# archi-physics/archi

Hardware: AMD Instinct MI355X
Metric: kNN queries/sec @ top-10, 10M x 768 bf16 corpus (higher is better)
Workload: dtype bf16

## Files before the change

### archi_amd/_lib.py

```python
from __future__ import annotations

import ctypes
import os
import threading

_HERE = os.path.dirname(os.path.abspath(__file__))
LIB_PATH = os.path.join(_HERE, "lib", "libarchi_hip.so")

DTYPES = {"f32": 0, "bf16": 1, "f16": 2}
METRICS = {"cosine": 0, "l2": 1, "inner_product": 2}
SEARCH_MODES = {"auto": 0, "exact": 1, "fast_only": 2}
POOLING = {"mean": 0, "cls": 1, "last": 2}


class HipBackendError(RuntimeError):
    """Raised when the HIP backend is unavailable or a call fails."""


class StaleFilterError(HipBackendError):
    """A search was handed a row_filter built for another layout of the index (AK_ERR_STALE_FILTER): a writer added rows
    or reclaimed tombstones between the mask's construction and the search. Rebuild the mask and retry."""


ERR_STALE_FILTER = -11
# ... 164 lines not shown
    ("ak_index_generate", _I, [_P, _U64, _U32, _U64, _I64, _I, _I64]),
    ("ak_index_remove", _I, [_P, _P, _I64, ctypes.POINTER(_I64)]),
    ("ak_index_count", _I, [_P, ctypes.POINTER(_I64)]),
    ("ak_index_fetch", _I, [_P, _P, _I64, _P]),
    ("ak_index_lookup", _I, [_P, _P, _I64, _P]),
    ("ak_index_distances", _I, [_P, _P, _P, _I64, _P, _P]),
    ("ak_index_search", _I, [_P, _P, _I, _I, _I, _P, _I64, _U64, _P, _P, _P, _P]),
    ("ak_index_lex_attach", _I, [_P, _P, _I64, _P, _P, _P, _P, _U64]),
    ("ak_index_lex_clear", _I, [_P, _U64]),
    ("ak_index_lex_info", _I, [_P, ctypes.POINTER(_U64), ctypes.POINTER(_I64), ctypes.POINTER(_I64), ctypes.POINTER(_I64)]),
    ("ak_index_lex_scores", _I, [_P, _P, _I, _D, _D, _D, _P, _P, _P]),
    ("ak_index_hybrid_search", _I, [_P, _P, _P, _I, _D, _D, _D, _D, _D, _P, _I64, _P, _I64, _U64, _I, _P, _P, ctypes.POINTER(_I),
                                    _P, _P, ctypes.POINTER(_I), _P]),
    ("ak_index_search_dev", _I, [_P, _P, _I, _I, _I, _P, _I64, _U64, _P, _P, _P, _P]),
    ("ak_index_slots", _I, [_P, ctypes.POINTER(_I64), ctypes.POINTER(_I64), ctypes.POINTER(_U64)]),
    ("ak_index_compact", _I, [_P, ctypes.POINTER(_I64)]),
    ("ak_index_scan_plan", _I, [_P, _I, _I, _P]),
    ("ak_index_i8_info", _I, [_P, _P]),
    ("ak_index_debug_read", _I, [_P, _P, _I]),
    ("ak_index_profile", _I, [_P, _I]),
    ("ak_index_profile_read", _I, [_P, _P, _I, ctypes.POINTER(_I)]),
    ("ak_merge_topk_dev", _I, [_I, _I, _I, _P, _P, _P, _P, _P]),
    ("ak_merge_shards_dev", _I, [_I, _I, _I, _P, _I64, _P, _P, _P, _P]),
    ("ak_comm_unique_id", _I, [_P]),
    ("ak_comm_create", _I, [_P, _I, _I, ctypes.POINTER(_P)]),
    ("ak_comm_destroy", _I, [_P]),
    ("ak_index_search_sharded_dev", _I, [_P, _P, _P, _I, _I, _P, _I64, _U64, _P, _P, ctypes.POINTER(_I64), _P]),
    ("ak_shard_payload_begin_dev", _I, [_P, _I, _I, _P]),
    ("ak_shard_fail_payload_dev", _I, [_P, _I, _I, _I, _P]),
    ("ak_shard_status_dev", _I, [_I, _P, _I64, _P, _P]),
    ("ak_shard_gather_rows_dev", _I, [_P, _P, _I, _I, _P, _P]),
    ("ak_shard_scatter_topk_dev", _I, [_P, _I, _I, _P, _P, _P, _P, _P]),
    ("ak_l2_normalize_dev", _I, [_P, _I64, _I, _P]),
    ("ak_encoder_create", _I, [ctypes.POINTER(AkBertConfig), _P, _I, ctypes.POINTER(_P)]),
    ("ak_encoder_destroy", _I, [_P]),
    ("ak_encoder_forward", _I, [_P, _P, _P, _I, _I, _I, _I, _P, _P]),
    ("ak_encoder_forward_lens", _I, [_P, _P, _I, _P, _I, _I, _I, _I, _I, _P, _P]),
    ("ak_encoder_gelu_table", _I, [_P]),
    ("ak_encoder_set_rel_bias", _I, [_P, _P, _I, _I]),
    ("ak_encoder_set_positions_from_ids", _I, [_P, _I, _I]),
    ("ak_decoder_create", _I, [ctypes.POINTER(AkDecoderConfig), _P, _I, ctypes.POINTER(_P)]),
    ("ak_decoder_destroy", _I, [_P]),
    ("ak_decoder_forward_lens", _I, [_P, _P, _I, _P, _I, _I, _I, _I, _P, _P]),
    ("ak_decoder_rope_table", _I, [ctypes.c_float, _I, _I, _P, _P]),
    ("ak_decoder_rope_table_inv", _I, [_P, _I, _I, _P, _P]),
    ("ak_mbert_create", _I, [ctypes.POINTER(AkModernBertConfig), _P, _I, ctypes.POINTER(_P)]),
    ("ak_mbert_destroy", _I, [_P]),
    ("ak_mbert_forward_lens", _I, [_P, _P, _I, _P, _I, _I, _I, _I, _I, _P, _P]),
    ("ak_gemma_create", _I, [ctypes.POINTER(AkGemmaConfig), _P, _I, ctypes.POINTER(_P)]),
    ("ak_gemma_destroy", _I, [_P]),
    ("ak_gemma_set_rope_inv_freq", _I, [_P, _P, _P]),
    ("ak_gemma_forward_lens", _I, [_P, _P, _I, _P, _I, _I, _I, _I, _I, _P, _P]),
    ("ak_nomic_create", _I, [ctypes.POINTER(AkNomicBertConfig), _P, _I, ctypes.POINTER(_P)]),
    ("ak_nomic_destroy", _I, [_P]),
    ("ak_nomic_forward_lens", _I, [_P, _P, _I, _P, _I, _I, _I, _I, _I, _P, _P]),
    ("ak_t5_create", _I, [ctypes.POINTER(AkT5Config), _P, _I, ctypes.POINTER(_P)]),
    ("ak_t5_destroy", _I, [_P]),
    ("ak_t5_forward_lens", _I, [_P, _P, _I, _P, _I, _I, _I, _I, _I, _P, _P]),
    ("ak_llama_create", _I, [ctypes.POINTER(AkLlamaConfig), _P, _I, ctypes.POINTER(_P)]),
    ("ak_llama_destroy", _I, [_P]),
    ("ak_llama_set_rope_inv_freq", _I, [_P, _P]),
    ("ak_llama_forward_lens", _I, [_P, _P, _I, _P, _I, _I, _I, _I, _I, _P, _P]),
    ("ak_qwen2_create", _I, [ctypes.POINTER(AkQwen2Config), _P, _I, ctypes.POINTER(_P)]),
    ("ak_qwen2_destroy", _I, [_P]),
    ("ak_qwen2_set_rope_inv_freq", _I, [_P, _P]),
    ("ak_qwen2_forward_lens", _I, [_P, _P, _I, _P, _I, _I, _I, _I, _I, _P, _P]),
    ("ak_wordpiece_create", _I, [ctypes.c_char_p, _I, ctypes.POINTER(_P)]),
    ("ak_wordpiece_create_ex", _I, [ctypes.c_char_p, _I, ctypes.c_char_p, ctypes.c_char_p, ctypes.c_char_p,
                                    ctypes.POINTER(ctypes.c_char_p), _I, ctypes.POINTER(_P)]),
    ("ak_wordpiece_destroy", _I, [_P]),
    ("ak_wordpiece_encode", _I, [_P, _P, _P, _I64, _I, _I, _P, _P]),
]


class AkKtGemm(ctypes.Structure):
    _fields_ = [
        ("X", _P), ("W", _P), ("bias", _P),
        ("T", _I), ("N", _I), ("K", _I),
        ("out_bf16", _P), ("ldo", _I),
        ("out_f32", _P),
        ("res16", _P),
        ("q", _P), ("k", _P), ("vt", _P), ("H", _I), ("S", _I), ("qscale", ctypes.c_float),
    ]


class AkKtGemmLazy(ctypes.Structure):
    _fields_ = [
        ("X", _P), ("W", _P), ("bias", _P),
        ("T", _I), ("N", _I), ("K", _I),
        ("out_bf16", _P), ("ldo", _I),
        ("res16", _P),
        ("q", _P), ("k", _P), ("vt", _P), ("H", _I), ("S", _I), ("qscale", ctypes.c_float),
        ("fold_c", _P), ("a_stats", _P), ("res_stats", _P), ("res_g", _P), ("res_b", _P), ("out_g", _P),
        ("out_stats", _P),
        ("nslot", _I), ("inv_h", ctypes.c_float), ("eps", ctypes.c_float),
    ]


KT_SYMBOLS = [
    ("ak_kt_attn", _I, [_P, _P, _P, _P, _P, _I, _I, _I, _I, _I, _I, _P, _P, _P, _I, _P]),
    ("ak_kt_attn_long", _I, [_P, _P, _P, _P, _P, _P, _I, _I, _I, _I, _I, _I, _P]),
    ("ak_kt_attn_window", _I, [_P, _P, _P, _P, _P, _P, _I, _I, _I, _I, _I, _I, _I, _P]),
    ("ak_kt_attn_causal", _I, [_P, _P, _P, _P, _P, _I, _I, _I, _I, _P]),
    ("ak_kt_gemm", _I, [_I, ctypes.POINTER(AkKtGemm), _P]),
    ("ak_kt_gemm_skinny", _I, [_P, _P, _P, _I, _I, _I, _P, _P, _I, _P]),
    ("ak_kt_gemm_skinny_qkv", _I, [_P, _P, _P, _I, _I, _I, _P, _P, _P, _I, _I, ctypes.c_float, _P]),
    ("ak_kt_vt_pos", _I, [_I]),
    ("ak_kt_gemm_ln", _I, [_P, _P, _P, _P, _P, _P, _P, _I, _I, ctypes.c_float, _P]),
    ("ak_kt_ffn384_weight_bytes", _I64, [_I]),
    ("ak_kt_ffn384", _I, [_P] * 13 + [_I, _I, ctypes.c_float, _P]),
    ("ak_kt_qkv384_weight_bytes", _I64, []),
    ("ak_kt_qkv384", _I, [_P] * 7 + [_I, _I, _I, ctypes.c_float, _I, _P]),
    ("ak_kt_gemm_lazy", _I, [_I, ctypes.POINTER(AkKtGemmLazy), _P]),
    ("ak_kt_ln_finalize", _I, [_P, _I, _I64, ctypes.c_float, ctypes.c_float, _P, _P]),
    ("ak_kt_fold_ln", _I, [_P, _P, _P, _P, _I, _I, _P, _P, _P]),
    ("ak_kt_layernorm", _I, [_P, _P, _P, _P, _P, _I, _I, ctypes.c_float, _P, _P, _P, _P]),
    ("ak_kt_layernorm16", _I, [_P, _P, _P, _I, _I, ctypes.c_float, _P, _P]),
    ("ak_kt_ln_apply16", _I, [_P, _P, _P, _P, _I64, _I, _P, _P]),
]

KTG_SYMBOLS = [
    ("ak_ktg_attn_gqa", _I, [_P, _P, _P, _P, _P, _I, _I, _I, _I, _I, _P]),
    ("ak_ktg_qk_norm_rope", _I, [_P, _I, _I, _I, _I, _P, _P, ctypes.c_float, _P, _P, ctypes.c_float, _P, _P, _P, _P]),
    ("ak_ktg_gemm_geglu_tanh", _I, [_P, _P, _P, _I, _I, _I, _P, _P]),
]

_F = ctypes.c_float
_EMBED = [_P, _I, _P, _I, _I, _I, _I, _I, _P, _P, _F, _P, _P]
KTS_SYMBOLS = [
    ("ak_kts_dec_embed", _I, _EMBED + [_P, _P]),
    ("ak_kts_dec_add_rmsnorm", _I, [_P, _P, _I64, _I, _P, _F, _P, _P]),
    ("ak_kts_dec_qk_rope", _I, [_P, _I, _I, _I, _I, _P, _P, _F, _P, _P, _F, _P, _P, _P, _P]),
    ("ak_kts_dec_pool", _I, [_P, _P, _I, _I, _I, _P, _F, _I, _P, _P]),
    ("ak_kts_mb_embed", _I, _EMBED + [_P, _P, _P]),
    ("ak_kts_mb_add_ln", _I, [_P, _P, _I64, _I, _P, _F, _P, _P]),
    ("ak_kts_mb_rope", _I, [_P, _P, _I64, _I, _I, _P, _P, _P]),
    ("ak_kts_mb_pool", _I, [_P, _P, _I, _I, _I, _F, _P, _I, _I, _P, _P, _P]),
    ("ak_kts_nb_embed", _I, [_P, _I, _P, _I, _I, _I, _I, _I, _P, _P, _P, _P, _F, _P, _P, _P, _P, _P]),
    ("ak_kts_nb_add_ln", _I, [_P, _P, _I64, _I, _P, _P, _F, _P, _P]),
    ("ak_kts_nb_pool", _I, [_P, _P, _I, _I, _I, _I, _I, _P, _P, _P]),
    ("ak_kts_gm_fold1p", _I, [_P, _I, _P, _P]),
    ("ak_kts_gm_embed", _I, _EMBED + [_P, _P]),
    ("ak_kts_gm_norm_add_norm", _I, [_P, _P, _I64, _I, _P, _P, _F, _P, _P, _P]),
    ("ak_kts_gm_pool", _I, [_P, _P, _I, _I, _I, _P, _P, _P]),
    ("ak_kts_gm_dense", _I, [_P, _P, _I, _I, _I, _P, _P]),
    ("ak_kts_gm_l2", _I, [_P, _I, _I, _I, _P, _P]),
    ("ak_kts_gemm_bf16", _I, [_P, _P, _P, _I, _I, _I, _P, _P]),
    ("ak_kts_ll_attn", _I, [_P, _P, _P, _P, _P, _I, _I, _I, _I, _I, _I, _P]),
    ("ak_kts_ll_pool", _I, [_P, _P, _I, _I, _I, _P, _F, _I, _P, _P, _P]),
    ("ak_kts_ll_rope", _I, [_P, _I, _I, _I, _I, _P, _P, _F, _P, _P, _P, _P]),
    ("ak_kts_q2_attn", _I, [_P, _P, _P, _P, _P, _I, _I, _I, _I, _I, _P]),
    ("ak_kts_t5_attn", _I, [_P, _P, _P, _P, _P, _P, _I, _I, _I, _I, _I, _I, _P, _I, _P]),
    ("ak_kts_t5_gemm_relu", _I, [_P, _P, _P, _I, _I, _I, _P, _P]),
]


def load() -> ctypes.CDLL:
    global _lib
    with _lock:
        if _lib is None:
            import torch
            path = LIB_PATH
            if os.environ.get("ARCHI_HIP_DBG") or any(os.environ.get(v) for v in DBG_SWITCHES) or \
                    os.environ.get("AK_SCAN_CFG", "")[:1] in ("X", "O") or os.environ.get("AK_ATTN_STREAM", "") in ("3", "4"):
                dbg = os.path.join(_HERE, "lib", "libarchi_hip_dbg.so")
                if not os.path.exists(dbg):
                    raise HipBackendError(f"{dbg} not found: the instrumented kernels are built by `make -C archi_amd/csrc dbg`")
                path = dbg
            if not os.path.exists(LIB_PATH):
                raise HipBackendError(
                    f"{LIB_PATH} not found: build it with `make -C archi_amd/csrc` "
                    "(or __graft_entry__.build()); archi_amd has no CPU fallback")
            lib = ctypes.CDLL(path)
            for name, res, args in SYMBOLS:
                fn = getattr(lib, name)
                fn.restype = res
                fn.argtypes = args
            if path != LIB_PATH:
                for name, res, args in KT_SYMBOLS + KTG_SYMBOLS + KTS_SYMBOLS:
                    fn = getattr(lib, name)
                    fn.restype = res
                    fn.argtypes = args
            got = lib.ak_abi_version()
            if got != ABI_VERSION:
                raise HipBackendError(f"{path}: ABI version {got}, this binding expects {ABI_VERSION} "
                                      "(rebuild with `make -C archi_amd/csrc`; signatures moved between the two)")
            _lib = lib
    return _lib


def is_dbg_library() -> bool:
    lib = load()
    return bool(getattr(lib, "_name", "").endswith("libarchi_hip_dbg.so"))


def debug_set(name: str, value: str | None) -> None:
    check(load().ak_debug_set(name.encode(), None if value is None else str(value).encode()), f"ak_debug_set({name})")


def last_error() -> str:
    return (load().ak_last_error() or b"").decode("utf-8", "replace")


def check(rc: int, what: str) -> None:
    if rc == ERR_STALE_FILTER:
        raise StaleFilterError(f"{what}: {last_error()}")
    if rc != 0:
        raise HipBackendError(f"{what} failed (rc={rc}): {last_error()}")


def init(device: int | None = None) -> ctypes.CDLL:
    global _inited_device
    lib = load()
    if device is None:
        device = int(os.environ.get("LOCAL_RANK", "0")) if _inited_device is None else _inited_device
    if _inited_device != device:
        check(lib.ak_init(device), "ak_init")
        _inited_device = device
    return lib


def bound_device() -> int:
    if _inited_device is None:
        raise HipBackendError("libarchi_hip is not initialised: call archi_amd._lib.init() first")
    return _inited_device
```

### archi_amd/csrc/exact.hip

```cpp
#include "index.h"
#include "switches.h"

namespace ak {

#pragma clang fp contract(off)

template <int DT>
__device__ inline void load8(const typename Store<DT>::T *row, int i, float (&v)[8]) {
    if constexpr (DT == AK_DTYPE_F32) {
        float4 a = *(const float4 *)(row + i), b = *(const float4 *)(row + i + 4);
        v[0] = a.x; v[1] = a.y; v[2] = a.z; v[3] = a.w; v[4] = b.x; v[5] = b.y; v[6] = b.z; v[7] = b.w;
    } else {
        uint4 u = *(const uint4 *)(row + i);
        const uint32_t w[4] = {u.x, u.y, u.z, u.w};
#pragma unroll
        for (int j = 0; j < 4; j++) {
            uint16_t lo = (uint16_t)(w[j] & 0xffffu), hi = (uint16_t)(w[j] >> 16);
            v[2 * j] = DT == AK_DTYPE_BF16 ? bf16_to_f32(lo) : f16_to_f32(lo);
            v[2 * j + 1] = DT == AK_DTYPE_BF16 ? bf16_to_f32(hi) : f16_to_f32(hi);
        }
    }
}

template <int DT>
__device__ inline double exact_distance(const typename Store<DT>::T *row, const float *q, int dim,
                                        int metric, float na, float nb) {
    using S = Store<DT>;
    const bool vec = (dim % 8 == 0) && (((uintptr_t)row & 15) == 0);
    float acc = 0.0f;
    if (metric == AK_METRIC_L2) {
        int i = 0;
        if (vec)
            for (; i < dim; i += 8) {
                float v[8];
                load8<DT>(row, i, v);
#pragma unroll
                for (int j = 0; j < 8; j++) {
                    float diff = __fsub_rn(v[j], q[i + j]);
                    acc = __fadd_rn(acc, __fmul_rn(diff, diff));
                }
            }
        for (; i < dim; i++) {
            float diff = __fsub_rn(S::load(row, i), q[i]);
            acc = __fadd_rn(acc, __fmul_rn(diff, diff));
        }
        return sqrt((double)acc);
    }
    int i = 0;
    if (vec)
        for (; i < dim; i += 8) {
            float v[8];
            load8<DT>(row, i, v);
#pragma unroll
            for (int j = 0; j < 8; j++) acc = __fadd_rn(acc, __fmul_rn(v[j], q[i + j]));
        }
    for (; i < dim; i++) acc = __fadd_rn(acc, __fmul_rn(S::load(row, i), q[i]));
    if (metric == AK_METRIC_IP) return (double)(-acc);
    double sim = (double)acc / sqrt((double)na * (double)nb);
    if (sim > 1.0) sim = 1.0;
    else if (sim < -1.0) sim = -1.0;
    return 1.0 - sim;
}

template <int DT, int QB>
__global__ __launch_bounds__(256) void k_exact_dist(const typename Store<DT>::T *__restrict__ rows,
                                                    const float *__restrict__ na,
                                                    const uint8_t *__restrict__ alive,
                                                    const uint8_t *__restrict__ filter, int64_t n, int dim,
                                                    int metric, const float *__restrict__ queries,
                                                    const float *__restrict__ nb, int nq,
                                                    uint64_t *__restrict__ keys) {
    using S = Store<DT>;
    int64_t r = (int64_t)blockIdx.x * blockDim.x + threadIdx.x;
    if (r >= n) return;
    bool ok = alive[r] && (!filter || filter[r]);
    if (!ok) {
        for (int qi = 0; qi < nq; qi++) keys[(int64_t)qi * n + r] = KEY_INVALID;
        return;
    }
    const typename S::T *row = rows + r * (int64_t)dim;
    float acc[QB];
#pragma unroll
    for (int qi = 0; qi < QB; qi++) acc[qi] = 0.0f;
    if (metric == AK_METRIC_L2) {
        for (int i = 0; i < dim; i++) {
            float a = S::load(row, i);
#pragma unroll
            for (int qi = 0; qi < QB; qi++) {
                float diff = __fsub_rn(a, queries[qi * dim + i]);
                acc[qi] = __fadd_rn(acc[qi], __fmul_rn(diff, diff));
            }
        }
    } else {
        for (int i = 0; i < dim; i++) {
            float a = S::load(row, i);
#pragma unroll
            for (int qi = 0; qi < QB; qi++)
                acc[qi] = __fadd_rn(acc[qi], __fmul_rn(a, queries[qi * dim + i]));
        }
    }
    float nar = na[r];
#pragma unroll
    for (int qi = 0; qi < QB; qi++) {
        if (qi >= nq) break;
        double d;
        if (metric == AK_METRIC_L2) d = sqrt((double)acc[qi]);
        else if (metric == AK_METRIC_IP) d = (double)(-acc[qi]);
        else {
            double sim = (double)acc[qi] / sqrt((double)nar * (double)nb[qi]);
            if (sim > 1.0) sim = 1.0;
            else if (sim < -1.0) sim = -1.0;
            d = 1.0 - sim;
        }
        keys[(int64_t)qi * n + r] = dist_key(d);
    }
}

__global__ __launch_bounds__(256) void k_query_norms(const float *__restrict__ q, int nq, int dim, float *__restrict__ nb) {
    __shared__ __attribute__((aligned(16))) float s_row[4][1024];
    const int wave = threadIdx.x >> 6, lane = threadIdx.x & 63;
    const int i = blockIdx.x * 4 + wave;
    if (i >= nq) return;
    const float *v = q + (int64_t)i * dim;
    float *row = s_row[wave];
    float s = 0.0f;
    for (int j0 = 0; j0 < dim; j0 += 1024) {
        const int len = dim - j0 < 1024 ? dim - j0 : 1024;
        for (int j = lane; j < len; j += 64) row[j] = v[j0 + j];
        __builtin_amdgcn_wave_barrier();
        __builtin_amdgcn_s_waitcnt(0xc07f);
        int j = 0;
        for (; j + 4 <= len; j += 4) {
            const float4 x = *(const float4 *)(row + j);
            s = __fadd_rn(s, __fmul_rn(x.x, x.x));
            s = __fadd_rn(s, __fmul_rn(x.y, x.y));
            s = __fadd_rn(s, __fmul_rn(x.z, x.z));
            s = __fadd_rn(s, __fmul_rn(x.w, x.w));
        }
        for (; j < len; j++) s = __fadd_rn(s, __fmul_rn(row[j], row[j]));
        __builtin_amdgcn_wave_barrier();
    }
    if (lane == 0) nb[i] = s;
}

int query_norms(const float *queries_dev, int nq, int dim, float *nb_dev, hipStream_t st) {
    if (nq <= 0) return 0;
    k_query_norms<<<(nq + 3) / 4, 256, 0, st>>>(queries_dev, nq, dim, nb_dev);
    AK_HIP(hipGetLastError());
    return 0;
}

template <int DT>
__global__ void k_rerank(const typename Store<DT>::T *__restrict__ rows, const float *__restrict__ na,
                         const int64_t *__restrict__ ids, int dim, int metric,
                         const float *__restrict__ queries, const float *__restrict__ nb, int nq, int kp,
                         const uint64_t *__restrict__ cand, uint64_t *__restrict__ okeys,
                         int64_t *__restrict__ oids) {
    int t = blockIdx.x * blockDim.x + threadIdx.x;
    if (t >= nq * kp) return;
    int qi = t / kp;
    uint64_t c = cand[t];
    if (c == KEY_INVALID) { okeys[t] = KEY_INVALID; oids[t] = -1; return; }
    int64_t r = (int64_t)(uint32_t)c;
    double d = exact_distance<DT>(rows + r * (int64_t)dim, queries + (int64_t)qi * dim, dim, metric, na[r],
                                  nb[qi]);
    okeys[t] = dist_key(d);
    oids[t] = ids[r];
}

int rerank(Index &ix, const float *queries_dev, const float *nb_dev, int nq, int kp, const uint64_t *cand,
           uint64_t *okeys, int64_t *oids, hipStream_t st) {
    int total = nq * kp;
    int grid = (total + 127) / 128;
#define LAUNCH(DT)                                                                                   \
    k_rerank<DT><<<grid, 128, 0, st>>>((const Store<DT>::T *)ix.rows, ix.na, ix.ids, ix.dim, ix.metric, \
                                       queries_dev, nb_dev, nq, kp, cand, okeys, oids)
    if (ix.dtype == AK_DTYPE_F32) LAUNCH(AK_DTYPE_F32);
    else if (ix.dtype == AK_DTYPE_BF16) LAUNCH(AK_DTYPE_BF16);
    else LAUNCH(AK_DTYPE_F16);
#undef LAUNCH
    AK_HIP(hipGetLastError());
    return 0;
}

constexpr int TL_THREADS = 256, TL_CAP = 2048, TL_PW = 64;

template <int DT>
__global__ __launch_bounds__(TL_THREADS) void k_tail(const typename Store<DT>::T *__restrict__ rows, const float *__restrict__ na,
                                                     const int64_t *__restrict__ ids, int dim, int metric,
                                                     const float *__restrict__ queries, const float *__restrict__ nb,
                                                     const uint64_t *__restrict__ list, int64_t lcap, const int *__restrict__ cnt_g,
                                                     const unsigned int *__restrict__ thr_g, const float *__restrict__ thr0,
                                                     const QPrep *__restrict__ prep, int k, int64_t *__restrict__ out_ids,
                                                     double *__restrict__ out_dist, int *__restrict__ out_cnt,
                                                     int *__restrict__ cert, int64_t *__restrict__ stats, int flags) {
    using S = Store<DT>;
    constexpr int KP = TAIL_KP, ES = (int)sizeof(typename S::T);
    constexpr int ROWB = TL_PW * ES;
    constexpr int STRIDE = ROWB + 16;
    constexpr int CPR = ROWB / 16;
    constexpr int CPT = KP * CPR / TL_THREADS;
    constexpr int SPP = 24 / CPT;
    constexpr int RAW = TL_CAP * 8 > 2 * KP * STRIDE ? TL_CAP * 8 : 2 * KP * STRIDE;
    __shared__ __attribute__((aligned(16))) char s_raw[RAW];
    __shared__ __attribute__((aligned(16))) float s_q[TAIL_MAX_DIM];
    __shared__ uint64_t s_top[KP];
    __shared__ uint64_t s_rk[KP];
    __shared__ int64_t s_ri[KP];
    __shared__ int s_n;
    uint64_t *s = (uint64_t *)s_raw;
    const int qi = blockIdx.x, tid = threadIdx.x, lane = tid & 63, wave = tid >> 6;
    float theta = thr0 ? thr0[qi] : -__builtin_inff();
    if (!(theta == theta)) theta = -__builtin_inff();
    const unsigned int tg = thr_g[qi];
    const float tmax = tg ? key_score(~tg) : -__builtin_inff();
    const float cutoff = tmax > theta ? tmax : theta;
    const uint32_t cut_key = score_key(cutoff);
    const int n = cnt_g[qi];
    if (tid == 0) s_n = 0;
    for (int i = tid; i < dim; i += TL_THREADS) s_q[i] = queries[(int64_t)qi * dim + i];
    __syncthreads();
    const uint64_t *lst = list + (int64_t)qi * lcap;
    for (int i = tid; i < n; i += TL_THREADS) {
        const uint64_t key = lst[i];
        if ((uint32_t)(key >> 32) <= cut_key) {
            const int pos = atomicAdd(&s_n, 1);
            if (pos < TL_CAP) s[pos] = key;
        }
    }
    __syncthreads();
    const int total = s_n;
    const bool overflow = total > TL_CAP;
    const int have = overflow ? TL_CAP : total;
    if (tid < KP) s_top[tid] = KEY_INVALID;
    __shared__ __attribute__((aligned(16))) uint64_t s_sel[2 * TL_THREADS + 4];
    __shared__ unsigned int s_hist[TL_THREADS];
    __shared__ unsigned int s_lo, s_hi;
    __shared__ int s_cutbin, s_ncut, s_nsel;
    const uint64_t *arr = s;
    uint64_t *arr_w = s;
    int cntv = have;
    bool by_count = have <= 2 * TL_THREADS;
    if (!by_count && !(flags & 1)) {
        static_assert(TL_THREADS == 256, "histogram cut: one bin per thread");
        if (tid == 0) { s_lo = 0xffffffffu; s_hi = 0u; s_nsel = 0; s_cutbin = 255; s_ncut = have; }
        s_hist[tid] = 0u;
        __syncthreads();
        unsigned int mylo = 0xffffffffu, myhi = 0u;
        for (int i = tid; i < have; i += TL_THREADS) {
            const unsigned int k32 = (unsigned int)(s[i] >> 32);
            mylo = k32 < mylo ? k32 : mylo; myhi = k32 > myhi ? k32 : myhi;
        }
        atomicMin(&s_lo, mylo); atomicMax(&s_hi, myhi);
        __syncthreads();
        const unsigned int lo = s_lo, range = s_hi - lo;
        const int shift = range < 256u ? 0 : (32 - __clz((int)range)) - 8;
        for (int i = tid; i < have; i += TL_THREADS) atomicAdd(&s_hist[((unsigned int)(s[i] >> 32) - lo) >> shift], 1u);
        __syncthreads();
        if (wave == 0) {
            unsigned int c[4], sum = 0;
#pragma unroll
            for (int j = 0; j < 4; j++) { c[j] = s_hist[lane * 4 + j]; sum += c[j]; }
            unsigned int incl = sum;
#pragma unroll
            for (int off = 1; off < 64; off <<= 1) { const unsigned int t = __shfl_up(incl, off); if (lane >= off) incl += t; }
            unsigned int run = incl - sum;
            int mybin = -1; unsigned int mycum = 0;
#pragma unroll
            for (int j = 0; j < 4; j++) { run += c[j]; if (mybin < 0 && run >= (unsigned int)KP) { mybin = lane * 4 + j; mycum = run; } }
            const uint64_t found = __ballot(mybin >= 0);
            if (found) {
                const int src = __builtin_ctzll(found);
                const int cb = __shfl(mybin, src); const unsigned int cc = __shfl(mycum, src);
                if (lane == 0) { s_cutbin = cb; s_ncut = (int)cc; }
            }
        }
        __syncthreads();
        const int ncut = s_ncut;
        if (ncut <= 2 * TL_THREADS) {
            const unsigned int cutbin = (unsigned int)s_cutbin;
            for (int i = tid; i < have; i += TL_THREADS) {
                const uint64_t key = s[i];
                if ((((unsigned int)(key >> 32) - lo) >> shift) <= cutbin) s_sel[atomicAdd(&s_nsel, 1)] = key;
            }
            arr = s_sel; arr_w = s_sel; cntv = ncut; by_count = true;
        }
    }
    if (by_count && !(flags & 1)) {
        __syncthreads();
        uint64_t mine[2];
        int rank[2] = {0, 0};
#pragma unroll
        for (int e = 0; e < 2; e++) mine[e] = tid + e * TL_THREADS < cntv ? arr[tid + e * TL_THREADS] : KEY_INVALID;
        const int cnt4 = (cntv + 3) & ~3;
        for (int j = cntv + tid; j < cnt4; j += TL_THREADS) arr_w[j] = KEY_INVALID;
        __syncthreads();
#pragma unroll 2
        for (int j = 0; j < cnt4; j += 4) {
            const uint4 a = *(const uint4 *)(arr + j), b = *(const uint4 *)(arr + j + 2);
            const uint64_t o0 = ((uint64_t)a.y << 32) | a.x, o1 = ((uint64_t)a.w << 32) | a.z,
                           o2 = ((uint64_t)b.y << 32) | b.x, o3 = ((uint64_t)b.w << 32) | b.z;
            rank[0] += (o0 < mine[0]) + (o1 < mine[0]) + (o2 < mine[0]) + (o3 < mine[0]);
            rank[1] += (o0 < mine[1]) + (o1 < mine[1]) + (o2 < mine[1]) + (o3 < mine[1]);
        }
#pragma unroll
        for (int e = 0; e < 2; e++)
            if (mine[e] != KEY_INVALID && rank[e] < KP) s_top[rank[e]] = mine[e];
        __syncthreads();
    } else {
        int m = KP;
        while (m < have) m <<= 1;
        for (int i = have + tid; i < m; i += TL_THREADS) s[i] = KEY_INVALID;
        __syncthreads();
        if (!(flags & 1))
        for (int size = 2; size <= m; size <<= 1) {
            for (int stride = size >> 1; stride > 0; stride >>= 1) {
                for (int t = tid; t < (m >> 1); t += TL_THREADS) {
                    const int p2 = 2 * t - (t & (stride - 1));
                    const uint64_t a = s[p2], b = s[p2 + stride];
                    const bool up = (p2 & size) == 0;
                    if ((a > b) == up) { s[p2] = b; s[p2 + stride] = a; }
                }
                __syncthreads();
            }
        }
        if (tid < KP) s_top[tid] = s[tid];
        __syncthreads();
    }
    const int valid_c = have < KP ? have : KP;
    const uint64_t last_c = s_top[KP - 1];

    float acc = 0.0f;
    const int npanels = dim / TL_PW;
    const char *rbase[CPT];
#pragma unroll
// ... 370 lines not shown
```

### archi_amd/csrc/index.h

```cpp
#pragma once
#include <atomic>
#include <condition_variable>
#include <mutex>
#include <shared_mutex>
#include <unordered_map>
#include <vector>

#include "coalesce.h"
#include "common.h"
#include "index_book.h"

namespace ak {

struct Workspace {
    void *buf = nullptr;
    size_t bytes = 0;
    int reserve(size_t need);
    void release();
};

struct Index : IndexBook {
    int dim = 0, dtype = 0, metric = 0;
    void *rows = nullptr;
    void *shadow = nullptr;
    float *na = nullptr, *ea = nullptr, *eb = nullptr;
    float *gb = nullptr;
    int64_t *ids = nullptr;
    uint8_t *alive = nullptr;
    int64_t *lex_off = nullptr;
    int32_t *lex_cnt = nullptr, *lex_len = nullptr;
    uint2 *lex_arena = nullptr;
    int64_t lex_arena_cap = 0, lex_used = 0;
    int64_t lex_entries = 0, lex_rows = 0;
    uint64_t lex_gen = 0;
    std::vector<int32_t> h_lex_cnt;
    std::vector<uint8_t> h_lex_att;
    Workspace ws_lex;
    std::mutex lex_mu;
    char *lex_pin = nullptr; size_t lex_pin_cap = 0;
    hipEvent_t lex_ev[5] = {nullptr, nullptr, nullptr, nullptr, nullptr};
    float max_na = 0.f;
    float max_rho = 0.f;
    int8_t *rows8 = nullptr;
    float *ea8 = nullptr, *gb8 = nullptr;
    int64_t s8_n = 0, s8_cap = 0;
    uint64_t s8_epoch = 0;
    float max_rho8 = 0.f;
    int64_t s8_builds = 0;
    std::atomic<int64_t> s8_searches{0};
    std::mutex s8_mu;
    Coalescer co;
    std::shared_mutex mu;
    Workspace ws_dev;
    Workspace ws_fb;
    std::mutex ws_mu;
    std::mutex prof_mu;
    hipEvent_t ws_event = nullptr;
    hipStream_t ws_stream = nullptr;
    bool ws_pending = false;
    float *max_dev = nullptr;
    long long *dbg_dev = nullptr;
    bool profile = false;
    std::vector<std::pair<hipEvent_t, hipEvent_t>> prof_events;
    size_t prof_used = 0;
};

size_t exact_scratch_bytes(const Index &ix, int k);
int exact_search(Index &ix, const float *queries_dev, const float *nb_dev, int nq, int k,
                 const uint8_t *filter_dev, int64_t *out_ids_dev, double *out_dist_dev,
                 int *out_cnt_dev, void *ws, hipStream_t st);

size_t select_scratch_bytes(int nq, int64_t n_in, int k);
int select_topk(const uint64_t *keys, const int64_t *ids, const int64_t *idmap, int nq, int64_t n_in,
                int k, uint64_t *okeys, int64_t *oids, void *scratch, hipStream_t st);

int select_topk_strided(const uint64_t *keys, int nq, int64_t n_in, int64_t in_stride, int k, uint64_t *okeys,
                        int64_t *oids, void *scratch, hipStream_t st);

size_t select_keys_scratch_bytes(int nq, int64_t n_in, int k);
int select_keys_topk(const uint64_t *keys, int nq, int64_t n_in, int64_t in_stride, int k, uint64_t *okeys,
                     void *scratch, hipStream_t st);

int rerank(Index &ix, const float *queries_dev, const float *nb_dev, int nq, int kp, const uint64_t *cand,
           uint64_t *okeys, int64_t *oids, hipStream_t st);

int query_norms(const float *queries_dev, int nq, int dim, float *nb_dev, hipStream_t st);

int emit_results(const uint64_t *keys, const int64_t *ids, int nq, int k, int64_t *out_ids,
                 double *out_dist, int *out_cnt, hipStream_t st);

int thread_stream(hipStream_t *out);
char *thread_scratch(size_t bytes);
void thread_scratch_trim();
int writer_fence(Index &ix);
int filter_is_current(const Index &ix, const void *row_filter, int64_t filter_len, uint64_t filter_epoch, const char *who);
int search_dev_locked(Index &ix, const float *queries_dev, int nq, int k, int mode, const uint8_t *row_filter_dev, int64_t *out_ids_dev,
                      double *out_dist_dev, int *out_cert_dev, hipStream_t st);
struct LexMove { int64_t *off = nullptr; int32_t *cnt = nullptr, *len = nullptr; };
int lex_rebuild(Index &ix, const LexMove &to, const std::vector<int64_t> *src, hipStream_t st, uint2 **new_arena, int64_t *new_cap,
                int64_t *new_used);
void lex_rebuilt(Index &ix, const std::vector<int64_t> *src, uint2 *new_arena, int64_t new_cap, int64_t new_used);
void lex_removed(Index &ix, const std::vector<int64_t> &slots);
void lex_release(Index &ix);

struct QPrep { double eps, a, b; };

int fused_tail(Index &ix, const float *queries_dev, const float *nb_dev, int nq, int k, const uint64_t *list, int64_t lcap,
               const int *cnt, const unsigned int *thr_max, const float *thr0, const QPrep *prep, int64_t *out_ids_dev,
               double *out_dist_dev, int *out_cnt_dev, int *cert_dev, int64_t *stats_dev, hipStream_t st);
constexpr int TAIL_KP = 64, TAIL_MAX_DIM = 4096;

struct FastPlan {
    int cfg;
    int kprime;
    int qtile;
    int nslices;
    int ns_seed;
    int64_t seed_rows;
    int64_t pre_tiles;
    int pre_slices;
    int pre_stride;
    int nqg;
    int i8;
    size_t bytes;
};
constexpr int AK_SHADOW8_NOMEM = -1008;
int ensure_shadow8(Index &ix, hipStream_t st);
void release_shadow8(Index &ix);
bool fast_supported(const Index &ix, int nq, int k);
FastPlan fast_plan(const Index &ix, int nq, int k, bool widest = false, bool allow_i8 = true);
int fast_search(Index &ix, const float *queries_dev, float *nb_dev, bool nb_ready, int nq, int k,
                const uint8_t *filter_dev, int64_t *out_ids_dev, double *out_dist_dev,
                int *out_cnt_dev, int *cert_dev, int64_t *stats_dev, void *ws, const FastPlan &plan,
                hipStream_t st);

}
```

### archi_amd/csrc/index.hip

```cpp
#include "index.h"
#include "switches.h"

#include <algorithm>
#include <atomic>
#include <cmath>
#include <cstring>
#include <limits>
#include <chrono>
#include <dlfcn.h>
#include <unordered_set>

namespace ak {

static thread_local std::string g_err;
void set_error(const std::string &msg) { g_err = msg; }

extern "C" char **environ;
static const std::unordered_map<std::string, std::string> &env_snapshot() {
    static const std::unordered_map<std::string, std::string> *snap = [] {
        auto *m = new std::unordered_map<std::string, std::string>();
        for (char **e = environ; e && *e; e++) {
            if (strncmp(*e, "AK_", 3) != 0) continue;
            const char *eq = strchr(*e, '=');
            if (eq) (*m)[std::string(*e, (size_t)(eq - *e))] = std::string(eq + 1);
        }
        return m;
    }();
    return *snap;
}
const char *env_get(const char *name) {
    const auto &m = env_snapshot();
    const auto it = m.find(name);
    return it == m.end() ? nullptr : it->second.c_str();
}
int env_int(const char *name, int dflt) {
    const char *e = env_get(name);
    return e && *e ? atoi(e) : dflt;
}
namespace {
struct SwitchName { const char *name; std::atomic<int> Switches::*field; int dflt; bool is_flag; bool wrong_results; bool is_char; };
const SwitchName g_switch_names[] = {
    {"AK_SCAN_CFG", &Switches::scan_cfg, 0, false, false, true},
    {"AK_SCAN_MFMA", &Switches::scan_mfma, 0, false, false, false},
    {"AK_SCAN_I8", &Switches::scan_i8, AK_SCAN_I8_DEFAULT, false, false, false},
    {"AK_SCAN_BLOCKS", &Switches::scan_blocks, 0, false, false, false},
    {"AK_SCAN_NO192", &Switches::scan_no192, 0, true, false, false},
    {"AK_SEED_RATIO", &Switches::seed_ratio, 32, false, false, false},
    {"AK_SEED_DIV", &Switches::seed_div, 0, false, false, false},
    {"AK_PRE_DIV", &Switches::pre_div, 0, false, false, false},
    {"AK_SCAN_NOSEED", &Switches::scan_noseed, 0, true, false, false},
    {"AK_SCAN_NOPRE", &Switches::scan_nopre, 0, true, false, false},
    {"AK_TAIL_OLD", &Switches::tail_old, 0, true, false, false},
    {"AK_SCAN_DBG", &Switches::scan_dbg, 0, true, false, false},
    {"AK_COALESCE_STATS", &Switches::coalesce_stats, 0, true, false, false},
    {"AK_SHARD_INJECT", &Switches::shard_inject, 0, false, false, false},
    {"AK_QUERY_FUSED", &Switches::query_fused, 0, false, false, false},
#if AK_DBG_KERNELS
    {"AK_SCAN_ABLATE", &Switches::scan_ablate, 0, false, true, false},
    {"AK_TAIL_ABLATE", &Switches::tail_ablate, 0, false, true, false},
#endif
};
int switch_value(const SwitchName &n, const char *v) {
    if (!v || !*v) return n.dflt;
    if (n.is_char) return (int)(unsigned char)v[0];
    if (n.is_flag) return 1;
    return atoi(v);
}
}
Switches &switches() {
    static Switches sw;
    static const bool once = [] {
        for (const SwitchName &n : g_switch_names) {
            if (n.wrong_results && !DBG_KERNELS) continue;
            (sw.*(n.field)).store(switch_value(n, env_get(n.name)), std::memory_order_relaxed);
        }
        if (const char *e = env_get("AK_SCAN_R192")) sw.scan_r192_pm.store((int)(atof(e) * 1000.0 + 0.5), std::memory_order_relaxed);
        return true;
    }();
    (void)once;
    return sw;
}
__attribute__((constructor)) static void ak_read_environment_at_load() { (void)switches(); }
int switches_set(const char *name, const char *value) {
    if (!name) return -1;
    Switches &sw = switches();
    if (!strcmp(name, "AK_SCAN_R192")) {
        sw.scan_r192_pm.store(value && *value ? (int)(atof(value) * 1000.0 + 0.5) : 850, std::memory_order_relaxed);
        return 0;
    }
    for (const SwitchName &n : g_switch_names)
        if (!strcmp(name, n.name)) {
            if (n.wrong_results && !DBG_KERNELS) return -1;
            if (!DBG_KERNELS && n.is_char && value && (*value == 'X' || *value == 'O')) return -1;
            if (!DBG_KERNELS && n.field == &Switches::scan_mfma && switch_value(n, value) != 0) return -1;
            if (n.field == &Switches::scan_mfma && switch_value(n, value) != 0 && switch_value(n, value) != 16 && switch_value(n, value) != 32) return -1;
            (sw.*(n.field)).store(switch_value(n, value), std::memory_order_relaxed);
            return 0;
        }
    return -1;
}

namespace {
struct RoctxApi {
    int (*push)(const char *) = nullptr;
    int (*pop)() = nullptr;
    RoctxApi() {
        for (const char *lib : {"librocprofiler-sdk-roctx.so.1", "librocprofiler-sdk-roctx.so", "libroctx64.so.4", "libroctx64.so"}) {
            if (void *h = dlopen(lib, RTLD_NOW | RTLD_GLOBAL)) {
                push = (int (*)(const char *))dlsym(h, "roctxRangePushA");
                pop = (int (*)())dlsym(h, "roctxRangePop");
                if (push && pop) return;
                push = nullptr; pop = nullptr;
            }
        }
    }
};
const RoctxApi &roctx() {
    static const RoctxApi api;
    return api;
}
}
RoctxRange::RoctxRange(const char *name) : on(roctx().push != nullptr) { if (on) roctx().push(name); }
RoctxRange::~RoctxRange() { if (on) roctx().pop(); }

int Workspace::reserve(size_t need) {
    if (need <= bytes) return 0;
    if (buf) hipFree(buf);
    buf = nullptr; bytes = 0;
    AK_HIP(hipMalloc(&buf, need));
    bytes = need;
    return 0;
}
void Workspace::release() {
    if (buf) hipFree(buf);
    buf = nullptr; bytes = 0;
}

constexpr size_t SCRATCH_KEEP = 256ull << 20;
struct ThreadCtx {
    hipStream_t stream = nullptr;
    char *dev = nullptr; size_t dev_cap = 0;
    char *ws = nullptr; size_t ws_cap = 0;
    char *pin = nullptr; size_t pin_cap = 0;
    void trim() {
        if (dev_cap > SCRATCH_KEEP) { hipFree(dev); dev = nullptr; dev_cap = 0; }
        if (ws_cap > SCRATCH_KEEP) { hipFree(ws); ws = nullptr; ws_cap = 0; }
        if (pin_cap > SCRATCH_KEEP) { hipHostFree(pin); pin = nullptr; pin_cap = 0; }
    }
    ~ThreadCtx() {
        if (ws) hipFree(ws);
        if (dev) hipFree(dev);
        if (pin) hipHostFree(pin);
        if (stream) hipStreamDestroy(stream);
    }
};
static std::atomic<int> g_device{-1};
static thread_local int t_bound_device = -1;
int bind_thread() {
    const int dev = g_device.load(std::memory_order_relaxed);
    if (dev >= 0 && t_bound_device != dev) {
        AK_HIP(hipSetDevice(dev));
        t_bound_device = dev;
    }
    return 0;
}

constexpr size_t CTX_POOL_MAX = 32;
static std::mutex g_ctx_mu;
static std::vector<ThreadCtx *> g_ctx_pool;
struct ThreadCtxHandle {
    ThreadCtx *p = nullptr;
    ThreadCtx &get() {
        if (!p) {
            {
                std::lock_guard<std::mutex> lk(g_ctx_mu);
                if (!g_ctx_pool.empty()) { p = g_ctx_pool.back(); g_ctx_pool.pop_back(); }
            }
            if (!p) p = new ThreadCtx();
        }
        return *p;
    }
    ~ThreadCtxHandle() {
        if (!p) return;
        {
            std::lock_guard<std::mutex> lk(g_ctx_mu);
            if (g_ctx_pool.size() < CTX_POOL_MAX) { g_ctx_pool.push_back(p); p = nullptr; }
        }
        delete p;
    }
};
static thread_local ThreadCtxHandle t_ctx_handle;
#define t_ctx (t_ctx_handle.get())
int thread_stream(hipStream_t *out) {
    if (!t_ctx.stream) AK_HIP(hipStreamCreateWithFlags(&t_ctx.stream, hipStreamNonBlocking));
    *out = t_ctx.stream;
    return 0;
}
static int scratch_reserve(char **p, size_t *cap, size_t need, bool pinned);
char *thread_scratch(size_t bytes) { return scratch_reserve(&t_ctx.dev, &t_ctx.dev_cap, bytes, false) ? nullptr : t_ctx.dev; }
void thread_scratch_trim() { t_ctx.trim(); }
static int scratch_reserve(char **p, size_t *cap, size_t need, bool pinned) {
    if (need <= *cap) return 0;
    if (*p) { if (pinned) hipHostFree(*p); else hipFree(*p); *p = nullptr; *cap = 0; }
    need = (need + 4095) & ~(size_t)4095;
    if (pinned) AK_HIP(hipHostMalloc((void **)p, need, hipHostMallocDefault));
// ... 1181 lines not shown
```

### archi_amd/csrc/switches.h

```cpp
#pragma once
#include <atomic>

#include "common.h"

namespace ak {

constexpr int AK_SCAN_I8_DEFAULT = 1;

struct Switches {
    std::atomic<int> scan_cfg{0};
    std::atomic<int> scan_mfma{0};
    std::atomic<int> scan_i8{AK_SCAN_I8_DEFAULT};
    std::atomic<int> scan_blocks{0};
    std::atomic<int> scan_r192_pm{850};
    std::atomic<int> scan_no192{0};
    std::atomic<int> seed_ratio{32};
    std::atomic<int> seed_div{0};
    std::atomic<int> pre_div{0};
    std::atomic<int> scan_noseed{0};
    std::atomic<int> scan_nopre{0};
    std::atomic<int> tail_old{0};
    std::atomic<int> scan_dbg{0};
    std::atomic<int> coalesce_stats{0};
    std::atomic<int> query_fused{0};
    std::atomic<int> shard_inject{0};
    std::atomic<int> scan_ablate{0};
    std::atomic<int> tail_ablate{0};
};
Switches &switches();
int switches_set(const char *name, const char *value);
const char *env_get(const char *name);
int env_int(const char *name, int dflt);
inline int dbg_env_int(const char *name, int dflt) { return DBG_KERNELS ? env_int(name, dflt) : dflt; }

}
```

Before: 117,300.

## Add LDS-staged panel rerank kernel with coalesced candidate row loads

Replaces the one-thread-per-candidate rerank, where each thread walks its own row with strided loads, with a wave-cooperative kernel. Each wave gathers 64 candidate rows in 128-byte panels using coalesced 16-byte loads, parks them in registers, stages them through LDS and then accumulates per-lane in the same sequential order, so exact distances stay bit-identical. The query is cached in LDS. It adds inline asm, LDS pressure and a dim%64 restriction, and keeps the old path behind AK_RERANK_OLD. Exports for a test harness are also added.

```diff
diff --git a/archi_amd/_lib.py b/archi_amd/_lib.py
--- a/archi_amd/_lib.py
+++ b/archi_amd/_lib.py
@@ -340,6 +340,8 @@
     ("ak_kts_q2_attn", _I, [_P, _P, _P, _P, _P, _I, _I, _I, _I, _I, _P]),
     ("ak_kts_t5_attn", _I, [_P, _P, _P, _P, _P, _P, _I, _I, _I, _I, _I, _I, _P, _I, _P]),
     ("ak_kts_t5_gemm_relu", _I, [_P, _P, _P, _I, _I, _I, _P, _P]),
+    ("ak_kts_rr_rerank", _I, [_P, _P, _I, _I, _P, _P, _P, _P, _I, _P]),
+    ("ak_kts_rr_choice", _I, [_P]),
 ]
 
 
diff --git a/archi_amd/csrc/exact.hip b/archi_amd/csrc/exact.hip
--- a/archi_amd/csrc/exact.hip
+++ b/archi_amd/csrc/exact.hip
@@ -20,6 +20,15 @@
             v[2 * j + 1] = DT == AK_DTYPE_BF16 ? bf16_to_f32(hi) : f16_to_f32(hi);
         }
     }
+}
+
+__device__ inline double exact_finish(float acc, int metric, float na, float nb) {
+    if (metric == AK_METRIC_L2) return sqrt((double)acc);
+    if (metric == AK_METRIC_IP) return (double)(-acc);
+    double sim = (double)acc / sqrt((double)na * (double)nb);
+    if (sim > 1.0) sim = 1.0;
+    else if (sim < -1.0) sim = -1.0;
+    return 1.0 - sim;
 }
 
 template <int DT>
@@ -44,7 +53,7 @@
             float diff = __fsub_rn(S::load(row, i), q[i]);
             acc = __fadd_rn(acc, __fmul_rn(diff, diff));
         }
-        return sqrt((double)acc);
+        return exact_finish(acc, metric, na, nb);
     }
     int i = 0;
     if (vec)
@@ -55,11 +64,7 @@
             for (int j = 0; j < 8; j++) acc = __fadd_rn(acc, __fmul_rn(v[j], q[i + j]));
         }
     for (; i < dim; i++) acc = __fadd_rn(acc, __fmul_rn(S::load(row, i), q[i]));
-    if (metric == AK_METRIC_IP) return (double)(-acc);
-    double sim = (double)acc / sqrt((double)na * (double)nb);
-    if (sim > 1.0) sim = 1.0;
-    else if (sim < -1.0) sim = -1.0;
-    return 1.0 - sim;
+    return exact_finish(acc, metric, na, nb);
 }
 
 template <int DT, int QB>
@@ -168,8 +173,143 @@
     oids[t] = ids[r];
 }
 
-int rerank(Index &ix, const float *queries_dev, const float *nb_dev, int nq, int kp, const uint64_t *cand,
-           uint64_t *okeys, int64_t *oids, hipStream_t st) {
+constexpr int RP_WAVES = 4, RP_THREADS = RP_WAVES * WAVE;
+constexpr int RP_ROWB = 128;
+constexpr int RP_STRIDE = RP_ROWB + 16;
+constexpr int RP_CPR = RP_ROWB / 16;
+constexpr int RP_CPL = WAVE * RP_CPR / WAVE;
+constexpr int RP_SPP = 24 / RP_CPL;
+constexpr int RP_IMAGE = WAVE * RP_STRIDE;
+
+template <int DT>
+__global__ __launch_bounds__(RP_THREADS) void k_rerank_panel(const typename Store<DT>::T *__restrict__ rows, const float *__restrict__ na,
+                                                             const int64_t *__restrict__ ids, int dim, int metric,
+                                                             const float *__restrict__ queries, const float *__restrict__ nb, int kp,
+                                                             int gpq, const uint64_t *__restrict__ cand, uint64_t *__restrict__ okeys,
+                                                             int64_t *__restrict__ oids) {
+    using S = Store<DT>;
+    constexpr int ES = (int)sizeof(typename S::T), PW = RP_ROWB / ES;
+    extern __shared__ __attribute__((aligned(16))) char s_dyn[];
+    float *s_q = (float *)s_dyn;
+    const int tid = threadIdx.x, lane = tid & 63, wave = tid >> 6;
+    const int qi = blockIdx.x / gpq, grp = blockIdx.x % gpq;
+    for (int i = tid; i < dim; i += RP_THREADS) s_q[i] = queries[(int64_t)qi * dim + i];
+    __syncthreads();
+    const int c0 = (grp * RP_WAVES + wave) * WAVE;
+    if (c0 >= kp) return;
+    const int ci = c0 + lane;
+    const int64_t t = (int64_t)qi * kp + ci;
+    const uint64_t key = ci < kp ? cand[t] : KEY_INVALID;
+    const bool valid = key != KEY_INVALID;
+    const uint64_t vmask = __ballot(valid);
+    if (!vmask) {
+        if (ci < kp) { okeys[t] = KEY_INVALID; oids[t] = -1; }
+        return;
+    }
+    const int slot = (int)(uint32_t)key;
+    const int spare = __shfl(slot, __builtin_ctzll(vmask));
+    const int fslot = valid ? slot : spare;
+    const char *rbase[RP_CPL];
+#pragma unroll
+    for (int j = 0; j < RP_CPL; j++)
+        rbase[j] = (const char *)rows + (int64_t)(uint32_t)__shfl(fslot, (lane >> 3) + 8 * j) * dim * ES + (lane & 7) * 16;
+    char *img = s_dyn + (size_t)dim * 4 + wave * RP_IMAGE;
+    char *wr = img + (lane >> 3) * RP_STRIDE + (lane & 7) * 16;
+    const char *row = img + lane * RP_STRIDE;
+    float acc = 0.0f;
+    const int npanels = dim / PW;
+    for (int p0 = 0; p0 < npanels; p0 += RP_SPP) {
+        const int np = npanels - p0 < RP_SPP ? npanels - p0 : RP_SPP;
+        uint4 park[RP_SPP][RP_CPL];
+#pragma unroll
+        for (int pp = 0; pp < RP_SPP; pp++)
+#pragma unroll
+            for (int j = 0; j < RP_CPL; j++) {
+                const char *g = rbase[j] + (int64_t)(p0 + (pp < np ? pp : np - 1)) * RP_ROWB;
+                asm volatile("global_load_dwordx4 %0, %1, off" : "=v"(park[pp][j]) : "v"(g) : "memory");
+            }
+        asm volatile("s_waitcnt vmcnt(0)" ::: "memory");
+#pragma unroll
+        for (int pp = 0; pp < RP_SPP; pp++)
+#pragma unroll
+            for (int j = 0; j < RP_CPL; j++)
+                asm volatile("" : "+v"(park[pp][j].x), "+v"(park[pp][j].y), "+v"(park[pp][j].z), "+v"(park[pp][j].w));
+#pragma unroll
+        for (int pp = 0; pp < RP_SPP; pp++) {
+            if (pp < np) {
+#pragma unroll
+                for (int j = 0; j < RP_CPL; j++) *(uint4 *)(wr + 8 * j * RP_STRIDE) = park[pp][j];
+                __builtin_amdgcn_wave_barrier();
+                __builtin_amdgcn_s_waitcnt(0xc07f);
+                if (valid) {
+                    const float *qq = s_q + (p0 + pp) * PW;
+#pragma unroll
+                    for (int i = 0; i < PW; i += 8) {
+                        float v[8];
+                        if constexpr (DT == AK_DTYPE_F32) {
+                            const float4 a = *(const float4 *)(row + i * 4), b = *(const float4 *)(row + i * 4 + 16);
+                            v[0] = a.x; v[1] = a.y; v[2] = a.z; v[3] = a.w; v[4] = b.x; v[5] = b.y; v[6] = b.z; v[7] = b.w;
+                        } else {
+                            const uint4 u = *(const uint4 *)(row + i * 2);
+                            const uint32_t w[4] = {u.x, u.y, u.z, u.w};
+#pragma unroll
+                            for (int e = 0; e < 4; e++) {
+                                const uint16_t lo = (uint16_t)(w[e] & 0xffffu), hi = (uint16_t)(w[e] >> 16);
+                                v[2 * e] = DT == AK_DTYPE_BF16 ? bf16_to_f32(lo) : f16_to_f32(lo);
+                                v[2 * e + 1] = DT == AK_DTYPE_BF16 ? bf16_to_f32(hi) : f16_to_f32(hi);
+                            }
+                        }
+                        if (metric == AK_METRIC_L2) {
+#pragma unroll
+                            for (int e = 0; e < 8; e++) {
+                                const float diff = __fsub_rn(v[e], qq[i + e]);
+                                acc = __fadd_rn(acc, __fmul_rn(diff, diff));
+                            }
+                        } else {
+#pragma unroll
+                            for (int e = 0; e < 8; e++) acc = __fadd_rn(acc, __fmul_rn(v[e], qq[i + e]));
+                        }
+                    }
+                }
+                __builtin_amdgcn_wave_barrier();
+            }
+        }
+    }
+    if (ci >= kp) return;
+    if (valid) {
+        const int64_t r = (int64_t)(uint32_t)key;
+        okeys[t] = dist_key(exact_finish(acc, metric, na[r], nb[qi]));
+        oids[t] = ids[r];
+    } else {
+        okeys[t] = KEY_INVALID;
+        oids[t] = -1;
+    }
+}
+
+bool rerank_panel_supported(const Index &ix) { return ix.dim > 0 && ix.dim % 64 == 0 && ix.dim <= TAIL_MAX_DIM; }
+bool rerank_takes_panel(const Index &ix) {
+    return rerank_panel_supported(ix) && !switches().rerank_old.load(std::memory_order_relaxed);
+}
+
+int rerank_with(Index &ix, const float *queries_dev, const float *nb_dev, int nq, int kp, const uint64_t *cand, uint64_t *okeys,
+                int64_t *oids, bool panel, hipStream_t st) {
+    if (nq <= 0 || kp <= 0) return 0;
+    if ((int64_t)nq * kp > 0x7fffffff) AK_FAIL(-1, "rerank: more than 2^31 candidates");
+    if (panel) {
+        if (!rerank_panel_supported(ix)) AK_FAIL(-1, "rerank: the panel kernel takes dim % 64 == 0, dim <= 4096");
+        const int gpq = (kp + RP_WAVES * WAVE - 1) / (RP_WAVES * WAVE);
+        if ((int64_t)nq * gpq > 0x7fffffff) AK_FAIL(-1, "rerank: too many workgroups");
+        const size_t lds = (size_t)ix.dim * 4 + RP_WAVES * RP_IMAGE;
+#define LAUNCH(DT)                                                                                                      \
+    k_rerank_panel<DT><<<nq * gpq, RP_THREADS, lds, st>>>((const Store<DT>::T *)ix.rows, ix.na, ix.ids, ix.dim, ix.metric, \
+                                                          queries_dev, nb_dev, kp, gpq, cand, okeys, oids)
+        if (ix.dtype == AK_DTYPE_F32) LAUNCH(AK_DTYPE_F32);
+        else if (ix.dtype == AK_DTYPE_BF16) LAUNCH(AK_DTYPE_BF16);
+        else LAUNCH(AK_DTYPE_F16);
+#undef LAUNCH
+        AK_HIP(hipGetLastError());
+        return 0;
+    }
     int total = nq * kp;
     int grid = (total + 127) / 128;
 #define LAUNCH(DT)                                                                                   \
@@ -181,6 +321,11 @@
 #undef LAUNCH
     AK_HIP(hipGetLastError());
     return 0;
+}
+
+int rerank(Index &ix, const float *queries_dev, const float *nb_dev, int nq, int kp, const uint64_t *cand,
+           uint64_t *okeys, int64_t *oids, hipStream_t st) {
+    return rerank_with(ix, queries_dev, nb_dev, nq, kp, cand, okeys, oids, rerank_takes_panel(ix), st);
 }
 
 constexpr int TL_THREADS = 256, TL_CAP = 2048, TL_PW = 64;
diff --git a/archi_amd/csrc/index.h b/archi_amd/csrc/index.h
--- a/archi_amd/csrc/index.h
+++ b/archi_amd/csrc/index.h
@@ -83,6 +83,10 @@
 
 int rerank(Index &ix, const float *queries_dev, const float *nb_dev, int nq, int kp, const uint64_t *cand,
            uint64_t *okeys, int64_t *oids, hipStream_t st);
+bool rerank_panel_supported(const Index &ix);
+bool rerank_takes_panel(const Index &ix);
+int rerank_with(Index &ix, const float *queries_dev, const float *nb_dev, int nq, int kp, const uint64_t *cand, uint64_t *okeys,
+                int64_t *oids, bool panel, hipStream_t st);
 
 int query_norms(const float *queries_dev, int nq, int dim, float *nb_dev, hipStream_t st);
 
diff --git a/archi_amd/csrc/index.hip b/archi_amd/csrc/index.hip
--- a/archi_amd/csrc/index.hip
+++ b/archi_amd/csrc/index.hip
@@ -51,6 +51,7 @@
     {"AK_SCAN_NOSEED", &Switches::scan_noseed, 0, true, false, false},
     {"AK_SCAN_NOPRE", &Switches::scan_nopre, 0, true, false, false},
     {"AK_TAIL_OLD", &Switches::tail_old, 0, true, false, false},
+    {"AK_RERANK_OLD", &Switches::rerank_old, 0, false, false, false},
     {"AK_SCAN_DBG", &Switches::scan_dbg, 0, true, false, false},
     {"AK_COALESCE_STATS", &Switches::coalesce_stats, 0, true, false, false},
     {"AK_SHARD_INJECT", &Switches::shard_inject, 0, false, false, false},
diff --git a/archi_amd/csrc/switches.h b/archi_amd/csrc/switches.h
--- a/archi_amd/csrc/switches.h
+++ b/archi_amd/csrc/switches.h
@@ -20,6 +20,7 @@
     std::atomic<int> scan_noseed{0};
     std::atomic<int> scan_nopre{0};
     std::atomic<int> tail_old{0};
+    std::atomic<int> rerank_old{0};
     std::atomic<int> scan_dbg{0};
     std::atomic<int> coalesce_stats{0};
     std::atomic<int> query_fused{0};
```

Measured after the change: 125,900, median of 6. +7.4%, better.
